# NoemieJaquier/GaBOtorch

Hardware: AMD Instinct MI355X
Metric: SPD affine-invariant kernel-matrix build, pairs/sec (N=4096,d=10) (higher is better)
Workload: dtype f64

## Files before the change

### gabotorch_amd/csrc/spd_pairwise_body.hpp

```cpp
#pragma once
#include "gabo_device.hpp"
#include "spd_eig.hpp"
#include "spd_prep.hpp"
#include "gabo_mirror.hpp"
#include "spd_generic.hpp"
#include "gabo_log_tab.hpp"
#include "gabo_exp_tab256.hpp"
#include "gabo_acosh2_table.hpp"
#include "../../include/gabo_hip.h"

#ifndef GABO_PAIR_WAVES
#define GABO_PAIR_WAVES 2
#endif

namespace gabo {

typedef const double __attribute__((address_space(1)))* spd_gcol_ptr;

struct SpdGcolBuffer {
    __amdgpu_buffer_rsrc_t rsrc;
    int voff;
    int stride_bytes;
    __device__ __forceinline__ double operator[](int k) const {
        return __builtin_bit_cast(double, __builtin_amdgcn_raw_buffer_load_b64(rsrc, voff, k * stride_bytes, 0));
    }
};
struct SpdGcolPointer {
    spd_gcol_ptr p;
    int64_t stride;
    __device__ __forceinline__ double operator[](int k) const { return p[(int64_t)k * stride]; }
};

template <int D, int ORIENT = kQlOrientPerLane, int CTL = kQlCtlPlain, class GCOL>
__device__ __forceinline__ double ai_sumsq(const double* __restrict__ W, const GCOL& Gj, const double* __restrict__ ltab, const double eps2 = 0.0) {
    constexpr int T = tri_size(D);
    constexpr bool kDescending = ORIENT == kQlOrientLast;
    double m[T];
    static_for<D>([&](auto cc) {
        constexpr int col = kDescending ? D - 1 - decltype(cc)::value : decltype(cc)::value;
        double g[D - col], c[D - col];
        static_for<D - col>([&](auto kk) { g[decltype(kk)::value] = Gj[tri(col + decltype(kk)::value, col)]; });
        static_for<D - col>([&](auto rr) {
            constexpr int r = col + decltype(rr)::value;
            double acc = W[tri(r, col)] * g[0];
            static_for<r - col>([&](auto kk) {
                constexpr int k = col + 1 + decltype(kk)::value;
                acc = __builtin_fma(W[tri(r, k)], g[k - col], acc);
            });
            c[r - col] = acc;
        });
        static_for<D - col>([&](auto rr) {
            constexpr int r = col + decltype(rr)::value;
            static_for<r - col + 1>([&](auto qq) {
                constexpr int q = col + decltype(qq)::value;
                m[tri(r, q)] = (kDescending ? col == q : col == 0) ? c[r - col] * c[q - col] : __builtin_fma(c[r - col], c[q - col], m[tri(r, q)]);
            });
        });
    });
    double dg[D], e2[D];
    tridiagonalize<D, ORIENT>(m, dg, e2);
    tridiag_eigenvalues<D, ORIENT, CTL>(dg, e2, eps2);
    double s = 0.0;
    const LogTabRegs lr = LogTabRegs::load();
    static_for<D>([&](auto kk) { double lg = log_tab(dg[decltype(kk)::value], lr, ltab); s = __builtin_fma(lg, lg, s); });
    return s;
}

struct Spd2Col {
    double g00, g10, g11, lg;
};
__device__ __forceinline__ double ai_sumsq2(const double* __restrict__ W, const Spd2Col& g, double lw, const LogTabRegs& lr,
                                            const double* __restrict__ ltab, double tiny) {
    const double c00 = W[0] * g.g00, c11 = W[2] * g.g11;
    const double c10 = __builtin_fma(W[1], g.g00, W[2] * g.g10);
    const double m00 = c00 * c00, m10d = (c10 + c10) * c00, m11 = __builtin_fma(c10, c10, c11 * c11);
    const double tr = m00 + m11, df = m00 - m11;
    const double root = sqrt_nz(__builtin_fma(df, df, __builtin_fma(m10d, m10d, tiny)));
    const double l1 = log_tab(0.5 * (tr + root), lr, ltab);
    const double l2 = __builtin_fma(2.0, lw + g.lg, -l1);
    return __builtin_fma(l1, l1, l2 * l2);
}

__device__ __forceinline__ double finish(double dist, double beta, int mode) {
    if (mode == GABO_OUT_DISTANCE) return dist;
    if (mode == GABO_OUT_LAPLACE) return exp(-(dist * beta));
    return exp(-((dist * dist) * beta));
}

#ifndef GABO_PAIR_TWO_WAVE_MAX_DIM
#define GABO_PAIR_TWO_WAVE_MAX_DIM 14
#endif
#ifndef GABO_QL_EPS2_GAUSS
#define GABO_QL_EPS2_GAUSS 1e-14
#endif
constexpr bool spd_pair_gauss_only_instantiated(int d) { return d > 2 && d != 12; }
#ifndef GABO_PAIR_ORIENT
constexpr int spd_pair_gauss_only_orientation(int d) { return d == 14 ? kQlOrientCol0 : kQlOrientLast; }
#else
constexpr int spd_pair_gauss_only_orientation(int d) { return GABO_PAIR_ORIENT; }
#endif
#ifndef GABO_PAIR_SWEEPCTL
constexpr int spd_pair_gauss_only_sweepctl(int d) { return d == 20 ? kQlCtlPlain : (kQlCtlDenormalZero | kQlCtlHwSqrt | kQlCtlStageThreshold); }
#else
constexpr int spd_pair_gauss_only_sweepctl(int d) { return GABO_PAIR_SWEEPCTL; }
#endif
template <int D, bool GAUSS_ONLY, bool BUFFER_ONLY>
__global__ __launch_bounds__(256, (D > GABO_PAIR_TWO_WAVE_MAX_DIM ? 1 : GABO_PAIR_WAVES)) void spd_ai_pairwise_kernel(const double* __restrict__ Winv, const double* __restrict__ G,
                                                              double* __restrict__ out, double* __restrict__ dist_out_arg,
                                                              int64_t n1, int64_t n2,
                                                              int64_t w_batch_stride, int64_t g_batch_stride, int rows,
                                                              int col_blocks, int row_chunks, int64_t sym_tiles, double beta, int flags) {
    constexpr int T = tri_size(D);
    static_assert(GAUSS_ONLY == BUFFER_ONLY && (spd_pair_gauss_only_instantiated(D) || !GAUSS_ONLY), "instantiations that launch_spd_ai selects");
    const int mode = GAUSS_ONLY ? GABO_OUT_GAUSSIAN : (flags & GABO_OUT_MASK);
    double* const dist_out = GAUSS_ONLY ? nullptr : dist_out_arg;
    constexpr bool kTabExp = D <= 4;
    __shared__ double tab[kTabExp ? 64 : 1];
    __shared__ __attribute__((aligned(16))) double ltab[512];
    for (int k = threadIdx.x; k < 512; k += blockDim.x) ltab[k] = kLogTab[k];
    double ec[6], ec3 = 0.0;
    if constexpr (kTabExp) {
        if (threadIdx.x < 64) tab[threadIdx.x] = kExp2Tab[threadIdx.x];
    }
    __syncthreads();
    if constexpr (kTabExp) {
        static_for<6>([&](auto k) { ec[decltype(k)::value] = kExpTabC[decltype(k)::value]; });
        ec3 = ec[3];
        asm volatile("" : "+v"(ec3));
    }
    int64_t cg, rc, b;
    if (flags & GABO_SYMMETRIC) {
        const int64_t per_batch = sym_tiles;
        b = blockIdx.x / per_batch;
        int64_t t = blockIdx.x - b * per_batch;
        cg = 0;
        for (;;) {
            int64_t cnt = ((cg + 1) * (int64_t)blockDim.x + rows - 1) / rows;
            if (cnt > row_chunks) cnt = row_chunks;
            if (t < cnt) break;
            t -= cnt;
            ++cg;
        }
        rc = t;
    } else {
        const int64_t bid = blockIdx.x;
        cg = bid % col_blocks;
        rc = (bid / col_blocks) % row_chunks;
        b = bid / ((int64_t)col_blocks * row_chunks);
    }
    const int64_t j0 = cg * blockDim.x;
    const int64_t j = j0 + threadIdx.x;
    const int64_t jc = j < n2 ? j : n2 - 1;
    const int64_t i0 = rc * rows;
    const int64_t i1 = (i0 + rows < n1) ? i0 + rows : n1;
    if ((flags & GABO_SYMMETRIC) && j0 + (int64_t)(threadIdx.x | 63) < i0) return;
    const double* Gj = G + b * g_batch_stride + jc;
    double* ob = out + b * n1 * n2;
    const int64_t jw = j0 + (threadIdx.x & ~63);
    const bool use_buffer = BUFFER_ONLY || (D > 2 && (int64_t)T * n2 * 8 < (1ll << 31));
    SpdGcolBuffer gbuf;
    {
        const double* gw = G + b * g_batch_stride + (jw < n2 ? jw : n2 - 1);
        uint64_t a = (uint64_t)gw;
        a = ((uint64_t)(uint32_t)__builtin_amdgcn_readfirstlane((int)(a >> 32)) << 32) | (uint32_t)__builtin_amdgcn_readfirstlane((int)a);
        gbuf.rsrc = __builtin_amdgcn_make_buffer_rsrc((void*)a, 0, 0x7fffffff, 0x00020000);
        gbuf.voff = (int)((jc - (jw < n2 ? jw : n2 - 1)) * 8);
        gbuf.stride_bytes = (int)(n2 * 8);
    }
    Spd2Col col2;
    double lw_lane = 0.0, tiny = 1e-290;
    LogTabRegs lr2;
    if constexpr (D == 2) {
        lr2 = LogTabRegs::load();
        asm volatile("" : "+s"(tiny));
        col2.g00 = Gj[0];
        col2.g10 = Gj[n2];
        col2.g11 = Gj[2 * n2];
        col2.lg = log_tab(col2.g00 * col2.g11, lr2, ltab);
        int64_t ir = i0 + (threadIdx.x & 63);
        ir = ir < n1 ? ir : n1 - 1;
        const double* Wr = Winv + b * w_batch_stride + ir * T;
        lw_lane = log_tab(Wr[0] * Wr[2], lr2, ltab);
    }
    double eps2 = (mode == GABO_OUT_GAUSSIAN && !dist_out) ? GABO_QL_EPS2_GAUSS : 0.0;
    asm volatile("" : "+s"(eps2));
    if constexpr (GAUSS_ONLY && BUFFER_ONLY) {
        const int nrows = __builtin_amdgcn_readfirstlane((int)(i1 - i0));
        const int64_t jrel = j - i0;
        const int rmax = j >= n2 ? -1 : ((flags & GABO_SYMMETRIC) ? (jrel < 0 ? -1 : (jrel > rows - 1 ? rows - 1 : (int)jrel)) : rows - 1);
        const double* W = Winv + b * w_batch_stride + i0 * T;
        char* orow = reinterpret_cast<char*>(ob + i0 * n2 + j);
        for (int r = 0; r < nrows; ++r, W += T) {
            SpdGcolBuffer gb = gbuf;
            asm volatile("" : "+v"(gb.voff));
            asm volatile("" : "+s"(gb.stride_bytes));
            const double s = ai_sumsq<D, spd_pair_gauss_only_orientation(D), spd_pair_gauss_only_sweepctl(D)>(W, gb, ltab, eps2);
            double val;
            if constexpr (kTabExp) {
                val = exp_neg_tab(-((s + 1e-15) * beta), ec, ec3, tab);
                val = s != s ? s : val;
            } else {
                val = exp(-((s + 1e-15) * beta));
            }
            if (r <= rmax) *reinterpret_cast<double*>(orow) = val;
            orow += (unsigned)gb.stride_bytes;
        }
        return;
    }
    for (int64_t i = i0; i < i1; ++i) {
        const double* W = Winv + b * w_batch_stride + i * T;
        double s;
        if constexpr (D == 2) {
            const int lane = (int)(i - i0);
            const double lw = __hiloint2double(__builtin_amdgcn_readlane(__double2hiint(lw_lane), lane),
                                               __builtin_amdgcn_readlane(__double2loint(lw_lane), lane));
            s = ai_sumsq2(W, col2, lw, lr2, ltab, tiny);
        } else {
            if (use_buffer) {
                SpdGcolBuffer gb = gbuf;
                asm volatile("" : "+v"(gb.voff));
                asm volatile("" : "+s"(gb.stride_bytes));
                s = ai_sumsq<D>(W, gb, ltab, eps2);
            } else {
                SpdGcolPointer gp{(spd_gcol_ptr)Gj, n2};
                asm volatile("" : "+v"(gp.p));
                s = ai_sumsq<D>(W, gp, ltab, eps2);
            }
        }
        double dist, val;
        if (mode == GABO_OUT_GAUSSIAN && !dist_out) {
            dist = 0.0;
            if constexpr (kTabExp) {
                val = exp_neg_tab(-((s + 1e-15) * beta), ec, ec3, tab);
                val = s != s ? s : val;
            } else {
                val = exp(-((s + 1e-15) * beta));
            }
        } else {
            dist = __builtin_sqrt(s + 1e-15);
            val = finish(dist, beta, mode);
        }
        if (j < n2 && (!(flags & GABO_SYMMETRIC) || i <= j)) {
            ob[i * n2 + j] = val;
            if (dist_out) dist_out[b * n1 * n2 + i * n2 + j] = dist;
        }
    }
}

#ifndef GABO_GAUSS2_MAX_ROWS
#define GABO_GAUSS2_MAX_ROWS 64
#endif
constexpr double kGauss2L = 0.0027076061740622863;
__constant__ double kGauss2C[6] = {kGauss2L, kGauss2L * kGauss2L / 2.0, kGauss2L * kGauss2L * kGauss2L / 6.0,
                                   kGauss2L * kGauss2L * kGauss2L * kGauss2L / 24.0, 6755399441055744.0, 4096.0};

template <bool NT, bool SYM>
__global__ __launch_bounds__(256) void spd_ai_gauss2_kernel(const double* __restrict__ Winv, const double* __restrict__ G,
                                                            double* __restrict__ out, int64_t n1, int64_t n2, int64_t w_batch_stride,
                                                            int64_t g_batch_stride, int rows, int col_blocks, int row_chunks,
                                                            int64_t sym_tiles, double beta, int flags) {
    __shared__ __attribute__((aligned(16))) double ltab[512];
    __shared__ double etab[256];
    __shared__ __attribute__((aligned(16))) double atab[kAcosh2Slots * kAcosh2Stride];
    __shared__ __attribute__((aligned(16))) double wrow[GABO_GAUSS2_MAX_ROWS * 4];
    const int tid = threadIdx.x;
    for (int k = tid; k < 512; k += blockDim.x) ltab[k] = kLogTab[k];
    for (int k = tid; k < 256; k += blockDim.x) etab[k] = kExp2Tab256[k];
    {
        const double sc = beta * (-512.0 / 0.69314718055994530942), eps = beta * (-256.0 / 0.69314718055994530942) * 1e-15;
        constexpr int kUsedLo = (kAcosh2Binades - 1) * 16 * kAcosh2Stride, kUsedHi = 240 * kAcosh2Stride;
        for (int k = tid; k < kAcosh2Slots * kAcosh2Stride - (kUsedHi - kUsedLo); k += blockDim.x) {
            const int kk = k < kUsedLo ? k : k + (kUsedHi - kUsedLo);
            const double v = kAcosh2Tab[kk] * sc;
            atab[kk] = (kk % kAcosh2Stride == 0) ? v + eps : v;
        }
    }
    int64_t cg, rc, b;
    if constexpr (SYM) {
        const int64_t per_batch = sym_tiles;
        b = blockIdx.x / per_batch;
        int64_t t = blockIdx.x - b * per_batch;
        cg = 0;
        for (;;) {
            int64_t cnt = ((cg + 1) * (int64_t)blockDim.x + rows - 1) / rows;
            if (cnt > row_chunks) cnt = row_chunks;
            if (t < cnt) break;
            t -= cnt;
            ++cg;
        }
        rc = t;
    } else {
        const int64_t bid = blockIdx.x;
        cg = bid % col_blocks;
        rc = (bid / col_blocks) % row_chunks;
        b = bid / ((int64_t)col_blocks * row_chunks);
    }
    const int64_t j0 = cg * blockDim.x;
    const int64_t j = j0 + tid;
    const int64_t jc = j < n2 ? j : n2 - 1;
    const int64_t i0 = rc * rows;
    const int64_t i1 = (i0 + rows < n1) ? i0 + rows : n1;
    const double* Gj = G + b * g_batch_stride + jc;
    const double g00 = Gj[0], g10 = Gj[n2], g11 = Gj[2 * n2];
    const LogTabRegs lr = LogTabRegs::load();
    const double sscale = __builtin_sqrt(beta * (512.0 / 0.69314718055994530942));
    double w0l = 1.0, w1l = 0.0, w2l = 1.0;
    if (tid < rows) {
        int64_t ir = i0 + tid;
        ir = ir < n1 ? ir : n1 - 1;
        const double* Wr = Winv + b * w_batch_stride + ir * 3;
        w0l = Wr[0], w1l = Wr[1], w2l = Wr[2];
    }
    __syncthreads();
    if (tid < rows) {
        const double dw = w0l * w2l;
        const double sw = rsqrt_nz(dw + dw);
        wrow[4 * tid + 0] = w0l * sw;
        wrow[4 * tid + 1] = w1l * sw;
        wrow[4 * tid + 2] = w2l * sw;
        wrow[4 * tid + 3] = sscale * log_tab(dw, lr, ltab);
    }
    __syncthreads();
    if (SYM && j0 + (int64_t)(tid | 63) < i0) return;
    double ec[6];
    static_for<6>([&](auto k) { ec[decltype(k)::value] = kGauss2C[decltype(k)::value]; });
    double c4v = ec[3];
    asm volatile("" : "+v"(c4v));
    const double dg = g00 * g11;
    const double bcol = sscale * log_tab(dg, lr, ltab);
    const double sg = rsqrt_nz(dg);
    const double q00 = g00 * sg, q10 = g10 * sg, q11 = g11 * sg;
    double* orow = out + b * n1 * n2 + i0 * n2 + j;
    const int nrows = __builtin_amdgcn_readfirstlane((int)(i1 - i0));
    const int64_t jrel = j - i0;
    const int rmax = j >= n2 ? -1 : (SYM ? (jrel < 0 ? -1 : (jrel > GABO_GAUSS2_MAX_ROWS - 1 ? GABO_GAUSS2_MAX_ROWS - 1 : (int)jrel)) : GABO_GAUSS2_MAX_ROWS - 1);
    typedef double g2_v2d __attribute__((ext_vector_type(2)));
    if (!SYM && j >= n2) return;
    for (int r = 0; r < nrows; ++r, orow += n2) {
        const g2_v2d wa = *reinterpret_cast<const g2_v2d*>(wrow + 4 * r);
        const g2_v2d wb = *reinterpret_cast<const g2_v2d*>(wrow + 4 * r + 2);
        const double w0 = wa[0], w1 = wa[1], w2 = wb[0], arow = wb[1];
        const double hh = __builtin_fma(w0, q00, -(w2 * q11));
        const double cc = __builtin_fma(w1, q00, w2 * q10);
        const double tau = __builtin_fma(cc, cc, __builtin_fma(hh, hh, 1.0));
        const unsigned hi = (unsigned)__double2hiint(tau);
        static_assert(kAcosh2MBits == 4 && kAcosh2Slots == 256, "row index = 8 bits");
        const unsigned off = __umul24((hi >> 16) & 0xffu, (unsigned)(kAcosh2Stride * sizeof(double)));
        const double t = tau - __hiloint2double((int)(hi & ~((1u << (20 - kAcosh2MBits)) - 1u)), 0);
        const g2_v2d* row = reinterpret_cast<const g2_v2d*>(reinterpret_cast<const char*>(atab) + off);
        static_assert(kAcosh2Deg == 7, "four coefficient pairs");
        const g2_v2d c67 = row[3], c45 = row[2], c23 = row[1], c01 = row[0];
        double ya = __builtin_fma(c67[1], t, c67[0]);
        ya = __builtin_fma(ya, t, c45[1]);
        ya = __builtin_fma(ya, t, c45[0]);
        ya = __builtin_fma(ya, t, c23[1]);
        ya = __builtin_fma(ya, t, c23[0]);
        ya = __builtin_fma(ya, t, c01[1]);
        ya = __builtin_fma(ya, t, c01[0]);
        if (__builtin_expect(__any(!(tau < ec[5])), 0)) {
            if (!(tau < ec[5])) {
                const double dl = log(tau + __builtin_sqrt(__builtin_fma(tau, tau, -1.0)));
                ya = -(sscale * sscale) * __builtin_fma(dl, dl, 0.5e-15);
            }
        }
        const double sp = arow + bcol;
        const double y = __builtin_fma(-sp, sp, ya);
        const double km = y + ec[4];
        const double kk = km - ec[4];
        const double rr = y - kk;
        double p = __builtin_fma(rr, c4v, ec[2]);
        p = __builtin_fma(p, rr, ec[1]);
        p = __builtin_fma(p, rr, ec[0]);
        p = p * rr;
        const int ki = __double2loint(km);
        const double e = etab[ki & 255];
        const double val = __builtin_ldexp(__builtin_fma(e, p, e), ki >> 8);
        if (!SYM || r <= rmax) {
            if constexpr (NT) __builtin_nontemporal_store(val, orow);
            else *orow = val;
        }
    }
}

template <int D>
static int launch_spd_ai(const double* x1, const double* x2, double* out, double* dist_out, int64_t batch, int64_t n1, int64_t n2,
                         int64_t s1, int64_t s2, double beta, int flags, double* ws, int* status, hipStream_t st, bool prepared = false) {
    constexpr int T = tri_size(D);
    const int64_t b1 = (s1 == 0) ? 1 : batch;
    const int64_t b2 = (s2 == 0) ? 1 : batch;
    double* W = ws;
    double* G = ws + b1 * n1 * T;
    if (!prepared) launch_spd_prep<D>(x1, x2, W, G, b1, b2, n1, n2, s1, s2, status, st, 1);
#ifndef GABO_PAIR_THREADS
#define GABO_PAIR_THREADS (D >= 7 ? 64 : 256)
#endif
    int threads = n2 >= 256 ? GABO_PAIR_THREADS : (n2 > 128 ? 192 : (n2 > 64 ? 128 : 64));
    int64_t col_blocks = (n2 + threads - 1) / threads;
#ifndef GABO_PAIR_ROWS_D2
#define GABO_PAIR_ROWS_D2 16
#endif
#ifndef GABO_PAIR_ROWS
#define GABO_PAIR_ROWS (D >= 9 ? 8 : 16)
#endif
#ifndef GABO_PAIR_ROWS_GAUSS2
#define GABO_PAIR_ROWS_GAUSS2 64
#endif
    const bool gauss2 = D == 2 && (flags & GABO_OUT_MASK) == GABO_OUT_GAUSSIAN && !dist_out && beta >= 0.0;
    int rows = D == 2 ? (gauss2 ? GABO_PAIR_ROWS_GAUSS2 : GABO_PAIR_ROWS_D2) : GABO_PAIR_ROWS;
    while (rows > 1 && col_blocks * ((n1 + rows - 1) / rows) * batch < (rows > 16 ? 1024 : 4096)) rows >>= 1;
    int64_t row_chunks = (n1 + rows - 1) / rows;
    int64_t sym_tiles = 0;
    if (flags & GABO_SYMMETRIC) {
        for (int64_t cg = 0; cg < col_blocks; ++cg) {
            int64_t cnt = ((cg + 1) * threads + rows - 1) / rows;
            sym_tiles += cnt < row_chunks ? cnt : row_chunks;
        }
    }
    int64_t nblocks = ((flags & GABO_SYMMETRIC) ? sym_tiles : col_blocks * row_chunks) * batch;
    if (nblocks > 0x7fffffffLL) return GABO_ERR_ARG;
    bool special2 = false;
    if constexpr (D == 2) special2 = gauss2 && rows <= GABO_GAUSS2_MAX_ROWS;
    if (special2) {
        const bool streaming = batch * n1 * n2 * 8 > (32ll << 20) && !(flags & GABO_SYMMETRIC);
#define GABO_GAUSS2_LAUNCH(...)                                                                                                     \
        hipLaunchKernelGGL((spd_ai_gauss2_kernel<__VA_ARGS__>), dim3((unsigned)nblocks), dim3(threads), 0, st, W, G, out, n1, n2,           \
                           (s1 == 0) ? (int64_t)0 : n1 * T, (s2 == 0) ? (int64_t)0 : n2 * T, rows, (int)col_blocks, (int)row_chunks,       \
                           sym_tiles, beta, flags)
        if (flags & GABO_SYMMETRIC) GABO_GAUSS2_LAUNCH(false, true);
        else if (streaming) GABO_GAUSS2_LAUNCH(true, false);
        else GABO_GAUSS2_LAUNCH(false, false);
#undef GABO_GAUSS2_LAUNCH
    } else {
#define GABO_PAIR_LAUNCH(...)                                                                                                             \
        hipLaunchKernelGGL((spd_ai_pairwise_kernel<D, __VA_ARGS__>), dim3((unsigned)nblocks), dim3(threads), 0, st, W, G, out, dist_out, n1, n2, \
                           (s1 == 0) ? (int64_t)0 : n1 * T, (s2 == 0) ? (int64_t)0 : n2 * T, rows, (int)col_blocks, (int)row_chunks,       \
                           sym_tiles, beta, flags)
        bool gauss_only = false;
        if constexpr (spd_pair_gauss_only_instantiated(D)) {
            gauss_only = (flags & GABO_OUT_MASK) == GABO_OUT_GAUSSIAN && !dist_out && (int64_t)T * n2 * 8 < (1ll << 31);
            if (gauss_only) GABO_PAIR_LAUNCH(true, true);
        }
        if (!gauss_only) GABO_PAIR_LAUNCH(false, false);
#undef GABO_PAIR_LAUNCH
    }
    if (flags & GABO_SYMMETRIC) {
        int tiles = (int)((n1 + 31) / 32);
        hipLaunchKernelGGL((mirror_upper_kernel<0>), dim3((unsigned)((int64_t)tiles * (tiles + 1) / 2), (unsigned)batch), dim3(256), 0, st,
                           out, n1, tiles);
        if (dist_out)
            hipLaunchKernelGGL((mirror_upper_kernel<0>), dim3((unsigned)((int64_t)tiles * (tiles + 1) / 2), (unsigned)batch), dim3(256), 0,
                               st, dist_out, n1, tiles);
    }
    return hipGetLastError() == hipSuccess ? GABO_OK : GABO_ERR_LAUNCH;
}

}

namespace gabo {
int launch_spd_ai_prepared(int d, double* out, int64_t batch, int64_t n1, int64_t n2, bool shared1, bool shared2, double beta, int flags,
                           double* ws, hipStream_t st);
int launch_spd_ai_wide2(int d, const double* x1, const double* x2, double* out, double* dist_out, int64_t batch, int64_t n1, int64_t n2,
                        int64_t s1, int64_t s2, double beta, int flags, double* ws, int* status, hipStream_t st);
int launch_spd_ai_wide3(int d, const double* x1, const double* x2, double* out, double* dist_out, int64_t batch, int64_t n1, int64_t n2,
                        int64_t s1, int64_t s2, double beta, int flags, double* ws, int* status, hipStream_t st);
int launch_spd_ai_wide(int d, const double* x1, const double* x2, double* out, double* dist_out, int64_t batch, int64_t n1, int64_t n2,
                       int64_t s1, int64_t s2, double beta, int flags, double* ws, int* status, hipStream_t st);
}
```

Before: 7.942 billion.

## Stage W and G loads ahead of congruence math for d=10 with three waves

For d=10 in the Gaussian-only path, the congruence product W·G is restructured into groups of W rows loaded via scalar (constant address space) loads, double-buffered, with G columns prefetched a fixed number of columns ahead, separated by explicit waitcnt and sched barriers. The launch bound raises the waves-per-EU hint to three for d=10, and the log-table constants are loaded through scalar constant memory to save VGPRs. The intent is to hide global load latency and raise occupancy. In exchange, the explicit waitcnt(0) barriers constrain scheduling and the tighter register budget may cause spills.

```diff
diff --git a/gabotorch_amd/csrc/spd_pairwise_body.hpp b/gabotorch_amd/csrc/spd_pairwise_body.hpp
--- a/gabotorch_amd/csrc/spd_pairwise_body.hpp
+++ b/gabotorch_amd/csrc/spd_pairwise_body.hpp
@@ -11,6 +11,8 @@
 
 #ifndef GABO_PAIR_WAVES
 #define GABO_PAIR_WAVES 2
+#else
+#define GABO_PAIR_WAVES_FORCED 1
 #endif
 
 namespace gabo {
@@ -31,11 +33,97 @@
     __device__ __forceinline__ double operator[](int k) const { return p[(int64_t)k * stride]; }
 };
 
-template <int D, int ORIENT = kQlOrientPerLane, int CTL = kQlCtlPlain, class GCOL>
+template <int D, int WLIM>
+struct SpdWGroups {
+    int n = 0;
+    int col[tri_size(D)] = {}, r0[tri_size(D)] = {}, r1[tri_size(D)] = {};
+    constexpr SpdWGroups() {
+        static_assert(WLIM >= D, "a row of the first column must fit a group");
+        for (int c = D - 1; c >= 0; --c) {
+            for (int r = c; r < D;) {
+                int sum = 0;
+                col[n] = c, r0[n] = r;
+                while (r < D && sum + (r - c + 1) <= WLIM) sum += r - c + 1, ++r;
+                r1[n++] = r;
+            }
+        }
+    }
+};
+#ifndef GABO_PAIR_WLIM
+#define GABO_PAIR_WLIM 16
+#endif
+template <int D, int AHEAD, class GCOL>
+__device__ __forceinline__ void ai_congruence_staged(const double* __restrict__ W, const GCOL& Gj, double (&m)[tri_size(D)]) {
+    constexpr SpdWGroups<D, (GABO_PAIR_WLIM < D ? D : GABO_PAIR_WLIM)> kG{};
+    double gq[D][D];
+    double wq[2][D][D];
+    double c[D];
+    auto issue_g = [&](auto ss) {
+        constexpr int col = D - 1 - decltype(ss)::value;
+        static_for<D - col>([&](auto kk) { gq[col][decltype(kk)::value] = Gj[tri(col + decltype(kk)::value, col)]; });
+    };
+    auto issue_w = [&](auto gg) {
+        constexpr int g = decltype(gg)::value, col = kG.col[g], r0 = kG.r0[g], r1 = kG.r1[g];
+        typedef const double __attribute__((address_space(4)))* wrow_ptr;
+        wrow_ptr Wg = (wrow_ptr)W;
+        asm volatile("" : "+s"(Wg));
+        static_for<r1 - r0>([&](auto rr) {
+            constexpr int r = r0 + decltype(rr)::value;
+            static_for<r - col + 1>([&](auto kk) { wq[g & 1][r][col + decltype(kk)::value] = Wg[tri(r, col + decltype(kk)::value)]; });
+        });
+    };
+    static_for<(AHEAD < D ? AHEAD : D)>(issue_g);
+    issue_w(std::integral_constant<int, 0>{});
+    static_for<kG.n>([&](auto gg) {
+        constexpr int g = decltype(gg)::value, col = kG.col[g], r0 = kG.r0[g], r1 = kG.r1[g];
+        if constexpr (r0 == col && D - 1 - col + AHEAD < D) issue_g(std::integral_constant<int, D - 1 - col + AHEAD>{});
+        __builtin_amdgcn_sched_barrier(0);
+        __builtin_amdgcn_s_waitcnt(0xc07f);
+        __builtin_amdgcn_sched_barrier(0);
+        if constexpr (g + 1 < kG.n) issue_w(std::integral_constant<int, g + 1>{});
+        static_for<r1 - r0>([&](auto rr) {
+            constexpr int r = r0 + decltype(rr)::value;
+            double acc = wq[g & 1][r][col] * gq[col][0];
+            static_for<r - col>([&](auto kk) {
+                constexpr int k = col + 1 + decltype(kk)::value;
+                acc = __builtin_fma(wq[g & 1][r][k], gq[col][k - col], acc);
+            });
+            c[r - col] = acc;
+        });
+        if constexpr (r1 == D) {
+            __builtin_amdgcn_sched_barrier(0);
+            static_for<D - col>([&](auto rr) {
+                constexpr int r = col + decltype(rr)::value;
+                static_for<r - col + 1>([&](auto qq) {
+                    constexpr int q = col + decltype(qq)::value;
+                    m[tri(r, q)] = col == q ? c[r - col] * c[q - col] : __builtin_fma(c[r - col], c[q - col], m[tri(r, q)]);
+                });
+            });
+        }
+    });
+    __builtin_amdgcn_sched_barrier(0);
+}
+
+__constant__ double kLogTabRegs[8] = {1.41421356237309504880, 1.0 / 7.0, -1.0 / 6.0, 0.2, -0.25, 1.0 / 3.0, 6.93147180369123816490e-01,
+                                      1.90821492927058770002e-10};
+__device__ __forceinline__ LogTabRegs log_tab_regs_scalar() {
+    typedef const double __attribute__((address_space(4)))* const_ptr;
+    const_ptr p = (const_ptr)kLogTabRegs;
+    asm volatile("" : "+s"(p));
+    LogTabRegs t;
+    t.sqrt2 = p[0], t.c7 = p[1], t.c6 = p[2], t.c5 = p[3], t.c4 = p[4], t.c3 = p[5], t.ln2_hi = p[6], t.ln2_lo = p[7];
+    return t;
+}
+
+template <int D, int ORIENT = kQlOrientPerLane, int CTL = kQlCtlPlain, int AHEAD = 0, class GCOL>
 __device__ __forceinline__ double ai_sumsq(const double* __restrict__ W, const GCOL& Gj, const double* __restrict__ ltab, const double eps2 = 0.0) {
     constexpr int T = tri_size(D);
     constexpr bool kDescending = ORIENT == kQlOrientLast;
     double m[T];
+    if constexpr (AHEAD > 0) {
+        static_assert(kDescending, "the staged congruence takes the columns from the last to the first");
+        ai_congruence_staged<D, AHEAD>(W, Gj, m);
+    } else
     static_for<D>([&](auto cc) {
         constexpr int col = kDescending ? D - 1 - decltype(cc)::value : decltype(cc)::value;
         double g[D - col], c[D - col];
@@ -61,7 +149,7 @@
     tridiagonalize<D, ORIENT>(m, dg, e2);
     tridiag_eigenvalues<D, ORIENT, CTL>(dg, e2, eps2);
     double s = 0.0;
-    const LogTabRegs lr = LogTabRegs::load();
+    const LogTabRegs lr = AHEAD > 0 ? log_tab_regs_scalar() : LogTabRegs::load();
     static_for<D>([&](auto kk) { double lg = log_tab(dg[decltype(kk)::value], lr, ltab); s = __builtin_fma(lg, lg, s); });
     return s;
 }
@@ -104,8 +192,18 @@
 #else
 constexpr int spd_pair_gauss_only_sweepctl(int d) { return GABO_PAIR_SWEEPCTL; }
 #endif
+#ifndef GABO_PAIR_WAVES_FORCED
+constexpr int spd_pair_gauss_only_waves(int d) { return d > GABO_PAIR_TWO_WAVE_MAX_DIM ? 1 : (d == 10 ? 3 : GABO_PAIR_WAVES); }
+#else
+constexpr int spd_pair_gauss_only_waves(int d) { return d > GABO_PAIR_TWO_WAVE_MAX_DIM ? 1 : GABO_PAIR_WAVES; }
+#endif
+#ifndef GABO_PAIR_AHEAD
+constexpr int spd_pair_gauss_only_ahead(int d) { return d == 10 && spd_pair_gauss_only_waves(d) == 3 ? 2 : 0; }
+#else
+constexpr int spd_pair_gauss_only_ahead(int d) { return d == 10 ? GABO_PAIR_AHEAD : 0; }
+#endif
 template <int D, bool GAUSS_ONLY, bool BUFFER_ONLY>
-__global__ __launch_bounds__(256, (D > GABO_PAIR_TWO_WAVE_MAX_DIM ? 1 : GABO_PAIR_WAVES)) void spd_ai_pairwise_kernel(const double* __restrict__ Winv, const double* __restrict__ G,
+__global__ __launch_bounds__(256, (GAUSS_ONLY ? spd_pair_gauss_only_waves(D) : (D > GABO_PAIR_TWO_WAVE_MAX_DIM ? 1 : GABO_PAIR_WAVES))) void spd_ai_pairwise_kernel(const double* __restrict__ Winv, const double* __restrict__ G,
                                                               double* __restrict__ out, double* __restrict__ dist_out_arg,
                                                               int64_t n1, int64_t n2,
                                                               int64_t w_batch_stride, int64_t g_batch_stride, int rows,
@@ -194,7 +292,7 @@
             SpdGcolBuffer gb = gbuf;
             asm volatile("" : "+v"(gb.voff));
             asm volatile("" : "+s"(gb.stride_bytes));
-            const double s = ai_sumsq<D, spd_pair_gauss_only_orientation(D), spd_pair_gauss_only_sweepctl(D)>(W, gb, ltab, eps2);
+            const double s = ai_sumsq<D, spd_pair_gauss_only_orientation(D), spd_pair_gauss_only_sweepctl(D), spd_pair_gauss_only_ahead(D)>(W, gb, ltab, eps2);
             double val;
             if constexpr (kTabExp) {
                 val = exp_neg_tab(-((s + 1e-15) * beta), ec, ec3, tab);
```

After: 8.134 billion, median of 6. 2.4% higher.
